# jing2li/MGPreconditionedGCR

Hardware: AMD Instinct MI355X
Metric: gcr_iterations_per_sec (higher is better)
Workload: dtype f64; 1 GPU; 3D 7-point Poisson 128^3 per GPU, unpreconditioned GCR restart 5, complex fp64, x0=0, RHS splitmix64 seed 0; rows=2097152, nnz=14581760, complex=True, stored_matrix_bytes=2097292, ell_width=7, tail_nnz=0, partition=1 GPU

## Files before the change

### mgpreconditionedgcr_amd/csrc/api.hip

```cpp
#include <algorithm>
#include <numeric>

#include <cstring>

#include "internal.h"

using namespace mgcr;

#define LOCK() std::lock_guard<std::recursive_mutex> lk__(ctx().mtx)

extern "C" {

int mgcr_csr_create(int64_t nrow, int64_t ncol, const int64_t *rowptr, const int64_t *col, const double *val_ri,
                    mgcr_op_t *out) {
    MGCR_TRY(require_ctx());
    MGCR_CHECK(out && rowptr && (col || rowptr[nrow] == 0) && (val_ri || rowptr[nrow] == 0), MGCR_ERR_INVALID,
               "mgcr_csr_create: null argument");
    LOCK();
    mgcr_op_s *op = new mgcr_op_s();
    op->kind = OP_CSR;
    op->dim = ncol;
    op->nrow = nrow;
    int rc = csr_build_device(nrow, ncol, rowptr, col, val_ri, &op->csr);
    if (rc != MGCR_OK) { delete op; return rc; }
// ... 168 lines not shown
    if (x_window) *x_window = o->csr.win_h;
    return MGCR_OK;
}

int mgcr_op_xr_fuse_kind(mgcr_op_t op, int32_t *kind) {
    MGCR_CHECK(op && kind, MGCR_ERR_INVALID, "mgcr_op_xr_fuse_kind: null argument");
    const Op *o = op_matrix(op);
    MGCR_CHECK(o->kind == OP_CSR, MGCR_ERR_UNSUPPORTED, "mgcr_op_xr_fuse_kind: not a Sparse");
    *kind = csr_fusable(o->csr, o->dist) ? csr_xr_fuse_kind(o->csr, o->dist) : 0;
    return MGCR_OK;
}

int mgcr_op_halo_kind(mgcr_op_t op, int32_t *kind) {
    MGCR_CHECK(op && kind, MGCR_ERR_INVALID, "mgcr_op_halo_kind: null argument");
    const Op *o = op_matrix(op);
    MGCR_CHECK(o->dist, MGCR_ERR_UNSUPPORTED, "mgcr_op_halo_kind: not a distributed Sparse");
    *kind = dist_halo_kind(o->dist);
    return MGCR_OK;
}

int mgcr_set_option(const char *name, int value, int *previous) {
    MGCR_CHECK(name, MGCR_ERR_INVALID, "null option name");
    if (!strcmp(name, "spmv_part")) {
        const int p = set_spmv_part(value);
        if (previous) *previous = p;
        return MGCR_OK;
    }
    bool prev;
    if (!strcmp(name, "pattern_storage")) prev = set_patterns_enabled(value != 0);
    else if (!strcmp(name, "stencil_storage")) prev = set_stencil_enabled(value != 0);
    else if (!strcmp(name, "lean_cycles")) prev = set_lean_enabled(value != 0);
    else if (!strcmp(name, "fused_apply")) prev = set_fuse_enabled(value != 0);
    else if (!strcmp(name, "graph_replay")) prev = set_graph_enabled(value != 0);
    else if (!strcmp(name, "resident_solver")) prev = set_resident_enabled(value != 0);
    else if (!strcmp(name, "step_build")) prev = set_stepbuild_enabled(value != 0);
    else if (!strcmp(name, "start_build")) prev = set_start_build_enabled(value != 0);
    else if (!strcmp(name, "step_build_keep_r")) {
        static bool last = true;
        prev = last;
        last = value != 0;
    }
    else if (!strcmp(name, "step_build_keep_all")) prev = set_stepbuild_keep_all_enabled(value != 0);
    else if (!strcmp(name, "halo_split")) prev = set_halo_split(value != 0);
    else if (!strcmp(name, "pw_tail")) prev = set_pw_tail_enabled(value != 0);
    else { set_error("mgcr_set_option: unknown option '%s'", name); return MGCR_ERR_INVALID; }
    if (previous) *previous = prev ? 1 : 0;
    return MGCR_OK;
}

int mgcr_stat(const char *name, int64_t *value) {
    MGCR_CHECK(name && value, MGCR_ERR_INVALID, "mgcr_stat: null argument");
    if (!strcmp(name, "resident_solves")) *value = resident_solve_count();
    else if (!strcmp(name, "step_build_launches")) *value = stepbuild_launch_count();
    else if (!strcmp(name, "start_build_launches")) *value = start_build_launch_count();
    else if (!strcmp(name, "small_solves")) *value = gcr_small_solve_count();
    else if (!strcmp(name, "one_launch_fallbacks")) *value = gcr_fallback_count();
    else if (!strcmp(name, "halo_split_exchanges")) *value = dist_halo_split_count();
    else if (!strcmp(name, "pw_tail_folds")) *value = comm_pw_tail_count();
    else if (!strcmp(name, "multi_solves")) *value = gcr_multi_solve_count();
    else if (!strcmp(name, "queue_solves")) *value = gcr_queue_stat(0);
    else if (!strcmp(name, "queue_admissions")) *value = gcr_queue_stat(1);
    else if (!strcmp(name, "queue_steps")) *value = gcr_queue_stat(2);
    else { set_error("mgcr_stat: unknown counter '%s'", name); return MGCR_ERR_INVALID; }
    return MGCR_OK;
}

int mgcr_selftest_coherence(int32_t steps, int32_t coherent, int64_t *rows_wrong) {
    MGCR_TRY(require_ctx());
    LOCK();
    return coherence_selftest(steps, coherent, rows_wrong);
}

int mgcr_op_stored_bytes(mgcr_op_t op, int64_t *matrix_bytes, int32_t *ell_width, int64_t *tail_nnz) {
    MGCR_CHECK(op, MGCR_ERR_INVALID, "null operator");
    const Op *o = op_matrix(op);
    if (o->kind == OP_CSR) {
        const CsrDev &A = o->csr;
        int64_t slab = (int64_t)A.nchunk * A.npad * A.L;
        int64_t ell_bytes = slab * (A.ell_val_re ? 12 : 20);
        if (csr_stencil_active(A)) ell_bytes = (A.npad / 64) * A.sten_stride * 8 + A.sten_kernel_ns * 20;
        else if (A.pat_mode == 1) ell_bytes = A.npad * 2 + (int64_t)A.npat * A.W * (A.pat_real ? 12 : 20);
        else if (A.pat_mode == 2) ell_bytes = A.npad * 2 + (int64_t)A.npat * A.W * 4 + slab * (A.ell_val_re ? 8 : 16);
        if (matrix_bytes) *matrix_bytes = ell_bytes + A.tail_nnz * 20 + A.n_tail_rows * 8 + (A.n_tail_rows ? 4 : 0);
        if (ell_width) *ell_width = A.nchunk * A.L;
        if (tail_nnz) *tail_nnz = A.tail_nnz;
        return MGCR_OK;
    }
    if (o->kind == OP_BCSR) {
        const BcsrDev &B = o->bcsr;
        if (matrix_bytes) *matrix_bytes = (int64_t)B.nblocks * (16LL * B.bs * B.bs + 4) + ((int64_t)B.nbrow + 1) * 4;
        if (ell_width) *ell_width = 0;
        if (tail_nnz) *tail_nnz = 0;
        return MGCR_OK;
    }
    set_error("mgcr_op_stored_bytes: not a matrix operator");
    return MGCR_ERR_UNSUPPORTED;
}

int mgcr_op_apply(mgcr_op_t op, mgcr_vec_t x, mgcr_vec_t y) {
    MGCR_TRY(require_ctx());
    MGCR_CHECK(op && x && y, MGCR_ERR_INVALID, "mgcr_op_apply: null argument");
    MGCR_REFUSE_MULTI_DIRAC(op, "mgcr_op_apply");
    MGCR_CHECK(x->n == op->dim, MGCR_ERR_INVALID, "Sparse matrix dimension does not match Field dimension!");
    int64_t nrow = op->nrow ? op->nrow : op->dim;
    MGCR_CHECK(y->n == nrow, MGCR_ERR_INVALID, "output Field has %lld entries, operator has %lld rows", (long long)y->n, (long long)nrow);
    MGCR_CHECK(x->d != y->d, MGCR_ERR_INVALID, "mgcr_op_apply: input and output must be different Fields");
// ... 233 lines not shown
```

### mgpreconditionedgcr_amd/csrc/gcr_stepbuild.hip

```cpp
#include <climits>
#include <cstdlib>
#include <type_traits>

#include "internal.h"
#include "reduce.h"
#include "gcr_dev.h"
#include "spmv_dev.h"
#include "exchange_dev.h"

namespace mgcr {

constexpr int SB_MAX_TRIPS = 4;
constexpr int SB_MAX_ND = 5;
constexpr int SB_KEEP_TB = 2;
template <int NDT> constexpr int sb_keep_rows() { return NDT == 1 ? 3 : 2; }
template <int NDT, bool XR, bool CLOSE> constexpr bool sb_close_merged() { return CLOSE && (NDT == 4 || (NDT == 5 && XR)); }

struct StepBuildArgs {
    RowMat m;
    const cplx *x;
    const cplx *aps[SB_MAX_ND];
    int64_t n;
    int nlogical;
    RowMap rm;
    DevState *st;
    int it;
    const double *partsR;
    int nblkR, strideR;
    double *hist;
    int hist_cap;
    const cplx *den;
    cplx *ap_out;
    double *partsA;
    LeanCoef *lc;
    const cplx *ps[SB_MAX_ND];
    cplx *p_out;
    cplx *xvec;
    cplx *xr_out;
    cplx *xr_den_slot;
    int xr_slot;
    double *partsR_out;
    v4i *slots;
    unsigned gen0;
    unsigned *abort_dev;
    int *abort_host;
    int spin_limit;
    int test_stall;
};

__device__ __forceinline__ cplx sb_xr_alpha(const ResSync &sy, DevState *st, LeanCoef *lc, cplx *xr_den_slot, int xr_slot, int lb) {
    const cplx num = make_double2(res_total(sy, 0), res_total(sy, 1)), den = make_double2(res_total(sy, 2), res_total(sy, 3));
    const cplx alpha = to_sgpr(cdiv(num, den));
    if (lb == 0 && threadIdx.x == 0) {
        *xr_den_slot = den;
        st->npend = xr_slot + 1;
    }
    if (lb == 0 && (int)threadIdx.x < LND) lean_pending_update(lc, xr_slot, alpha, (int)threadIdx.x);
    return alpha;
}

template <int MODE, int WT, int NDT, bool XR, bool CLOSE, bool REALC = false>
__global__ void __launch_bounds__(RED_THREADS, 8) step_build_kernel(StepBuildArgs a) {
    __shared__ double lds[(2 * NDT > 4 ? 2 * NDT : 4) * 17];
    __shared__ double lds_pw[2 * SB_MAX_ND * 17], lds_ws[2 * SB_MAX_ND * RES_GRP];
    __shared__ int gave_up;
    __shared__ cplx sbeta[NDT], scp[NDT];
    extern __shared__ __attribute__((aligned(16))) unsigned char sb_smem[];
    if (a.st->stop_at < a.st->base + a.it) return;
// ... 153 lines not shown
        }
        __builtin_amdgcn_sched_barrier(0);
    };
    if constexpr (XR) {
        if ((int)threadIdx.x < 4) {
            const v4i w4 = {__double2loint(mine), __double2hiint(mine), (int)sy.gen, 0};
            __builtin_amdgcn_raw_buffer_store_b128(w4, sy.slots, ((2 * RES_NV + (int)threadIdx.x) * RES_BLK + lb) * 16, 0, RES_SC1);
        }
        if constexpr (MERGED) close_last();
        const cplx xr0 = i0 < end ? a.x[i0] : make_double2(0., 0.);
        if (!res_collect<4>(sy, 2)) {
            res_abort(a.abort_dev, a.abort_host);
            for (int64_t i = i0; i < end; i += stride) a.xr_out[i] = make_double2(__builtin_nan(""), __builtin_nan(""));
            if (threadIdx.x == 0) a.partsR_out[lb] = __builtin_nan("");
            return;
        }
        if (ends_here) return;
        const cplx alpha = sb_xr_alpha(sy, a.st, a.lc, a.xr_den_slot, a.xr_slot, lb);
        double vr[1] = {0.};
        trip = 0;
        for (int64_t i = i0; i < end; i += stride, trip++) {
            const cplx rn = csub(i == i0 ? xr0 : a.x[i], cmul(alpha, arL[trip * RED_THREADS + (int)threadIdx.x]));
            a.xr_out[i] = rn;
            vr[0] += rn.x * rn.x + rn.y * rn.y;
        }
        const double tot = block_sum_owner<1>(vr, lds);
        if (threadIdx.x == 0) a.partsR_out[lb] = tot;
    }
}

template <class T>
__device__ __forceinline__ T *sb_elem(T *p, uint32_t off) {
    using C = std::conditional_t<std::is_const_v<T>, const char, char>;
    return reinterpret_cast<T *>(reinterpret_cast<C *>(p) + off);
}

__device__ __forceinline__ void sb_wave_pair_to_lds(double (&v)[2], double *lds, int k0) {
    double s;
    const int k = wave_multi_sum<2>(v, s);
    if (((int)threadIdx.x & 31) == 0) lds[(k0 + k) * 17 + ((int)threadIdx.x >> 6)] = s;
}
template <int NV>
__device__ __forceinline__ double sb_block_owner_from_lds(double *lds) {
    const int nwave = (blockDim.x + 63) >> 6;
    __syncthreads();
    double t = 0.;
    if (threadIdx.x < NV)
        for (int w = 0; w < nwave; w++) t += lds[threadIdx.x * 17 + w];
    return t;
}

template <int NDT, bool XR, bool CLOSE, bool REALC>
__global__ void __launch_bounds__(RED_THREADS, 8) step_keep_kernel(StepBuildArgs a) {
    __shared__ double lds[(2 * NDT > 4 ? 2 * NDT : 4) * 17];
    __shared__ double lds_pw[2 * SB_MAX_ND * 17], lds_ws[2 * SB_MAX_ND * RES_GRP];
    __shared__ int gave_up;
    __shared__ cplx sbeta[NDT], scp[NDT], scx[NDT];
    extern __shared__ __attribute__((aligned(16))) unsigned char sb_smem[];
    if (a.st->stop_at < a.st->base + a.it) return;
    const int lb = logical_workgroup(a.rm, (int)blockIdx.x, (int)gridDim.x);
    if (lb >= a.nlogical) return;
    cplx *arL = reinterpret_cast<cplx *>(sb_smem);
    const int tid = (int)threadIdx.x;
    ResSync sy;
    res_sync_init(sy, a.slots, a.gen0, a.nlogical, lb, a.abort_dev, a.spin_limit, lds_pw, lds_ws, &gave_up);
    if (a.test_stall && lb == a.test_stall - 1) return;
    int64_t i0, end, stride;
    row_range(a.rm, lb, a.nlogical, a.n, &i0, &end, &stride);
    auto row = [&](int t) -> int64_t { return i0 + (int64_t)t * stride; };
    uint32_t off[SB_MAX_TRIPS];
#pragma unroll
    for (int t = 0; t < SB_MAX_TRIPS; t++) off[t] = (uint32_t)row(t) * (uint32_t)sizeof(cplx);
    auto at = [&](auto *p, int t) { return sb_elem(p, off[t]); };
    cplx rk[SB_MAX_TRIPS];
#pragma unroll
    for (int t = 0; t < SB_MAX_TRIPS; t++) {
        const int64_t i = row(t);
        rk[t] = make_double2(0., 0.);
        if (i < end) {
            const PatLds pl{nullptr, nullptr, nullptr};
            cplx sum;
            const auto xj = [&](int32_t j) -> cplx { return *sb_elem(a.x, (uint32_t)j * (uint32_t)sizeof(cplx)); };
            if constexpr (REALC) sum = sten_row_product_t<7, false, 1>(a.m, i, xj);
            else sum = fused_row_product<3, 7>(a.m, i, 0, pl, xj);
            rk[t] = *at(a.x, t);
            arL[t * RED_THREADS + tid] = a.m.shift ? csub(rk[t], cmul(a.m.k, sum)) : sum;
        }
        __builtin_amdgcn_sched_barrier(0);
    }
    constexpr int KT = sb_keep_rows<NDT>();
    cplx pre[KT];
    {
#pragma unroll
        for (int jj = 0; jj < NDT; jj++) {
            const int j = NDT - 1 - jj;
            cplx b[SB_MAX_TRIPS];
#pragma unroll
            for (int t = 0; t < SB_MAX_TRIPS; t++) b[t] = row(t) < end ? ld_stream<true>(at(a.aps[j], t)) : make_double2(0., 0.);
            double v[2] = {0., 0.};
#pragma unroll
            for (int t = 0; t < SB_MAX_TRIPS; t++) {
                if (row(t) < end) {
                    const cplx tt = cconj_mul(arL[t * RED_THREADS + tid], b[t]);
                    v[0] += tt.x;
                    v[1] += tt.y;
                }
            }
            if (j == 0) {
#pragma unroll
                for (int u = 0; u < KT; u++) pre[u] = b[u];
            }
            sb_wave_pair_to_lds(v, lds, 2 * j);
            __builtin_amdgcn_sched_barrier(0);
        }
        const double mine = sb_block_owner_from_lds<2 * NDT>(lds);
        if (tid < 2 * NDT) {
            const v4i w4 = {__double2loint(mine), __double2hiint(mine), (int)sy.gen, 0};
            __builtin_amdgcn_raw_buffer_store_b128(w4, sy.slots, ((1 * RES_NV + tid) * RES_BLK + lb) * 16, 0, RES_SC1);
        }
    }
    if (!res_collect<2 * NDT>(sy, 1)) {
        res_abort(a.abort_dev, a.abort_host);
        for (int64_t i = i0; i < end; i += stride) a.ap_out[i] = make_double2(__builtin_nan(""), __builtin_nan(""));
        if (tid < 4) a.partsA[tid * RED_MAX_BLOCKS + lb] = __builtin_nan("");
        return;
    }
    bool ends_here = false;
    if (XR || lb == 0) {
        double rr[1];
        fold_partials<1>(a.partsR, a.nblkR, a.strideR, rr, lds);
        if (lb == 0 && threadIdx.x == 0) {
            close_step(a.st, a.it, rr[0], a.hist, a.hist_cap, CLOSE);
            if (CLOSE) a.st->closed = 1;
        }
        ends_here = __builtin_amdgcn_readfirstlane(!((rr[0] / a.st->bnorm2) > a.st->tol2)) != 0;
    }
    if (tid < NDT) sbeta[tid] = cdiv(make_double2(res_total(sy, 2 * tid), res_total(sy, 2 * tid + 1)), a.den[tid]);
    __syncthreads();
    if constexpr (CLOSE) {
        if (tid < NDT) {
            scp[tid] = lean_close_coef(a.lc, sbeta, NDT, tid);
            scx[tid] = a.lc->cx[tid];
        }
        __syncthreads();
    }
    if (!CLOSE && lb == 0 && tid <= NDT) lean_table_row<NDT>(a.lc, sbeta, tid);
    {
        cplx beta[NDT];
#pragma unroll
        for (int j = 0; j < NDT; j++) beta[j] = to_sgpr(sbeta[j]);
        double v[4] = {0., 0., 0., 0.};
#pragma unroll
        for (int t0 = 0; t0 < SB_MAX_TRIPS; t0 += SB_KEEP_TB) {
            cplx ac[SB_KEEP_TB];
#pragma unroll
            for (int u = 0; u < SB_KEEP_TB; u++) ac[u] = make_double2(0., 0.);
#pragma unroll
            for (int j = 0; j < NDT; j++) {
                cplx aj[SB_KEEP_TB];
#pragma unroll
                for (int u = 0; u < SB_KEEP_TB; u++)
                    aj[u] = (j == 0 && t0 + u < KT) ? pre[t0 + u < KT ? t0 + u : 0]
                            : row(t0 + u) < end   ? ld_stream<NTS>(at(a.aps[j], t0 + u))
                                                  : make_double2(0., 0.);
#pragma unroll
                for (int u = 0; u < SB_KEEP_TB; u++) ac[u] = csub(ac[u], cmul(beta[j], aj[u]));
                __builtin_amdgcn_sched_barrier(0);
            }
#pragma unroll
            for (int u = 0; u < SB_KEEP_TB; u++) {
                const int t = t0 + u;
                const int64_t i = row(t);
                if (i < end) {
                    const cplx an = cadd(arL[t * RED_THREADS + tid], ac[u]);
                    *at(a.ap_out, t) = an;
                    if (XR) arL[t * RED_THREADS + tid] = an;
                    const cplx tt = cconj_mul(rk[t], an);
                    v[0] += tt.x; v[1] += tt.y;
                    const cplx w = cconj_mul(an, an);
                    v[2] += w.x; v[3] += w.y;
                }
            }
        }
        const double mine = block_sum_owner<4>(v, lds);
        if (tid < 4) a.partsA[tid * RED_MAX_BLOCKS + lb] = mine;
        if (XR && tid < 4) {
            const v4i w4 = {__double2loint(mine), __double2hiint(mine), (int)sy.gen, 0};
            __builtin_amdgcn_raw_buffer_store_b128(w4, sy.slots, ((2 * RES_NV + tid) * RES_BLK + lb) * 16, 0, RES_SC1);
        }
    }
    if constexpr (CLOSE) {
        cplx cx[NDT], cp[NDT];
#pragma unroll
        for (int j = 0; j < NDT; j++) {
            cx[j] = to_sgpr(scx[j]);
            cp[j] = to_sgpr(scp[j]);
        }
#pragma unroll
        for (int t0 = 0; t0 < SB_MAX_TRIPS; t0 += SB_KEEP_TB) {
            cplx xv[SB_KEEP_TB], pc[SB_KEEP_TB];
#pragma unroll
            for (int u = 0; u < SB_KEEP_TB; u++) {
                xv[u] = row(t0 + u) < end ? *at(a.xvec, t0 + u) : make_double2(0., 0.);
                pc[u] = make_double2(0., 0.);
            }
#pragma unroll
            for (int j = 0; j < NDT; j++) {
                cplx pj[SB_KEEP_TB];
#pragma unroll
                for (int u = 0; u < SB_KEEP_TB; u++) pj[u] = row(t0 + u) < end ? ld_stream<NTS>(at(a.ps[j], t0 + u)) : make_double2(0., 0.);
#pragma unroll
                for (int u = 0; u < SB_KEEP_TB; u++) {
                    xv[u] = cadd(xv[u], cmul(cx[j], pj[u]));
                    pc[u] = csub(pc[u], cmul(cp[j], pj[u]));
                }
            }
#pragma unroll
            for (int u = 0; u < SB_KEEP_TB; u++) {
                const int64_t i = row(t0 + u);
                if (i < end) {
                    *at(a.xvec, t0 + u) = xv[u];
                    st_stream<NTS>(at(a.p_out, t0 + u), cadd(rk[t0 + u], pc[u]));
                }
            }
            __builtin_amdgcn_sched_barrier(0);
        }
    }
    if constexpr (XR) {
        if (!res_collect<4>(sy, 2)) {
            res_abort(a.abort_dev, a.abort_host);
            for (int64_t i = i0; i < end; i += stride) a.xr_out[i] = make_double2(__builtin_nan(""), __builtin_nan(""));
            if (threadIdx.x == 0) a.partsR_out[lb] = __builtin_nan("");
            return;
        }
        if (ends_here) return;
        const cplx alpha = sb_xr_alpha(sy, a.st, a.lc, a.xr_den_slot, a.xr_slot, lb);
        double vr[1] = {0.};
#pragma unroll
        for (int t = 0; t < SB_MAX_TRIPS; t++) {
            const int64_t i = row(t);
            if (i < end) {
                const cplx rn = csub(rk[t], cmul(alpha, arL[t * RED_THREADS + tid]));
                *at(a.xr_out, t) = rn;
                vr[0] += rn.x * rn.x + rn.y * rn.y;
            }
        }
        const double tot = block_sum_owner<1>(vr, lds);
        if (threadIdx.x == 0) a.partsR_out[lb] = tot;
    }
}

struct StartArgs {
    RowMat m;
    const cplx *b;
    cplx *ap0;
    int64_t n;
    int nlogical;
    RowMap rm;
    DevState *st;
    double *hist;
    LeanCoef *lc;
    cplx *den0;
    cplx *r_out;
    double *partsR_out;
    v4i *slots;
    unsigned gen0;
    unsigned *abort_dev;
    int *abort_host;
    int spin_limit;
    int test_stall;
};

template <bool REALC>
__global__ void __launch_bounds__(RED_THREADS, 8) start_build_kernel(StartArgs a) {
    __shared__ double lds[6 * 17];
    __shared__ double lds_pw[2 * SB_MAX_ND * 17], lds_ws[2 * SB_MAX_ND * RES_GRP];
    __shared__ int gave_up;
    extern __shared__ __attribute__((aligned(16))) unsigned char sb_smem[];
    if (a.st->stop_at < 0) return;
    const int lb = logical_workgroup(a.rm, (int)blockIdx.x, (int)gridDim.x);
    if (lb >= a.nlogical) return;
    cplx *apL = reinterpret_cast<cplx *>(sb_smem);
    ResSync sy;
    res_sync_init(sy, a.slots, a.gen0, a.nlogical, lb, a.abort_dev, a.spin_limit, lds_pw, lds_ws, &gave_up);
    if (a.test_stall && lb == a.test_stall - 1) return;
    int64_t i0, end, stride;
    row_range(a.rm, lb, a.nlogical, a.n, &i0, &end, &stride);
    {
        double v[6] = {0., 0., 0., 0., 0., 0.};
#pragma unroll
        for (int t = 0; t < SB_MAX_TRIPS; t++) {
            const int64_t i = i0 + (int64_t)t * stride;
            if (i < end) {
                const PatLds pl{nullptr, nullptr, nullptr};
                cplx sum;
                if constexpr (REALC) sum = sten_row_product_t<7, false, 1>(a.m, i, [&](int32_t j) -> cplx { return a.b[j]; });
                else sum = fused_row_product<3, 7>(a.m, i, 0, pl, [&](int32_t j) -> cplx { return a.b[j]; });
                const cplx rv = a.b[i];
                const cplx yi = a.m.shift ? csub(rv, cmul(a.m.k, sum)) : sum;
                a.ap0[i] = yi;
                apL[t * RED_THREADS + (int)threadIdx.x] = yi;
                v[4] += rv.x * rv.x + rv.y * rv.y;
                const cplx tt = cconj_mul(rv, yi);
                v[0] += tt.x; v[1] += tt.y;
                const cplx u = cconj_mul(yi, yi);
                v[2] += u.x; v[3] += u.y;
            }
            __builtin_amdgcn_sched_barrier(0);
        }
        const double mine = block_sum_owner<6>(v, lds);
        if ((int)threadIdx.x < 5) {
            const v4i w4 = {__double2loint(mine), __double2hiint(mine), (int)sy.gen, 0};
            __builtin_amdgcn_raw_buffer_store_b128(w4, sy.slots, ((1 * RES_NV + (int)threadIdx.x) * RES_BLK + lb) * 16, 0, RES_SC1);
        }
    }
    const cplx b0 = i0 < end ? a.b[i0] : make_double2(0., 0.);
    if (!res_collect<5>(sy, 1)) {
        res_abort(a.abort_dev, a.abort_host);
        for (int64_t i = i0; i < end; i += stride) a.r_out[i] = make_double2(__builtin_nan(""), __builtin_nan(""));
        if (threadIdx.x == 0) a.partsR_out[lb] = __builtin_nan("");
        return;
    }
    if (lb == 0 && threadIdx.x == 0) {
        const double nb = res_total(sy, 4);
        a.st->bnorm2 = nb;
        a.st->rr = nb;
        a.hist[0] = sqrt(nb) / sqrt(nb);
    }
    const cplx alpha = sb_xr_alpha(sy, a.st, a.lc, a.den0, 0, lb);
    double vr[1] = {0.};
#pragma unroll
    for (int t = 0; t < SB_MAX_TRIPS; t++) {
        const int64_t i = i0 + (int64_t)t * stride;
        if (i < end) {
            const cplx rn = csub(t == 0 ? b0 : a.b[i], cmul(alpha, apL[t * RED_THREADS + (int)threadIdx.x]));
            a.r_out[i] = rn;
            vr[0] += rn.x * rn.x + rn.y * rn.y;
        }
    }
    const double tot = block_sum_owner<1>(vr, lds);
    if (threadIdx.x == 0) a.partsR_out[lb] = tot;
}

static EnvSwitch g_stepbuild{"MGCR_STEPBUILD"}, g_start_build{"MGCR_START_BUILD"};
static EnvSwitch g_sb_keep_all{"MGCR_SB_KEEP_ALL"};
static EnvSwitch g_sb_real{"MGCR_SB_REAL"};
bool stepbuild_is_enabled() { return g_stepbuild.on(); }
bool set_stepbuild_enabled(bool on) { return g_stepbuild.set(on); }
bool set_start_build_enabled(bool on) { return g_start_build.set(on); }
bool set_stepbuild_keep_all_enabled(bool on) { return g_sb_keep_all.set(on); }
static int64_t g_stepbuild_launches = 0;
int64_t stepbuild_launch_count() { return g_stepbuild_launches; }

template <int NDT, bool XR, bool CLOSE> constexpr bool sb_keep_fits() { return NDT <= 2 || (NDT == 3 && !(XR && CLOSE)); }
template <int NDT, bool XR, bool CLOSE, bool R> const void *sb_keep() {
    if constexpr (sb_keep_fits<NDT, XR, CLOSE>()) return (const void *)step_keep_kernel<NDT, XR, CLOSE, R>;
    else return nullptr;
}
static const void *sb_kernel(int nd, bool xr, bool close, bool realc) {
    if (g_sb_keep_all.on() && nd <= 3) {
#define SKR(NDT, R) (close ? (xr ? sb_keep<NDT, true, true, R>() : sb_keep<NDT, false, true, R>()) \
                           : (xr ? sb_keep<NDT, true, false, R>() : sb_keep<NDT, false, false, R>()))
#define SKK(NDT) (realc ? SKR(NDT, true) : SKR(NDT, false))
        const void *keep = nd == 1 ? SKK(1) : nd == 2 ? SKK(2) : SKK(3);
#undef SKK
#undef SKR
        if (keep) return keep;
    }
#define SBR(NDT, R) (close ? (xr ? (const void *)step_build_kernel<3, 7, NDT, true, true, R> : (const void *)step_build_kernel<3, 7, NDT, false, true, R>) \
                           : (xr ? (const void *)step_build_kernel<3, 7, NDT, true, false, R> : (const void *)step_build_kernel<3, 7, NDT, false, false, R>))
#define SBK(NDT) (realc ? SBR(NDT, true) : SBR(NDT, false))
    switch (nd) {
        case 1: return SBK(1);
        case 2: return SBK(2);
        case 3: return SBK(3);
        case 4: return SBK(4);
        default: return SBK(5);
    }
#undef SBK
#undef SBR
}
bool launch_is_coresident(const void *kernel, int threads, size_t dyn_lds, int grid) {
    struct Key { const void *k; size_t lds; int threads; int per_cu; };
    static std::vector<Key> seen;
    int per_cu = -1;
    for (const Key &e : seen)
        if (e.k == kernel && e.lds == dyn_lds && e.threads == threads) per_cu = e.per_cu;
    if (per_cu < 0) {
        if (dyn_lds > 0) (void)hipFuncSetAttribute(kernel, hipFuncAttributeMaxDynamicSharedMemorySize, (int)(dyn_lds > 64 * 1024 ? dyn_lds : 64 * 1024));
        int nb = 0;
        if (hipOccupancyMaxActiveBlocksPerMultiprocessor(&nb, kernel, threads, dyn_lds) != hipSuccess) { (void)hipGetLastError(); nb = 0; }
        per_cu = nb;
        seen.push_back(Key{kernel, dyn_lds, threads, per_cu});
    }
    static const int force = getenv("MGCR_TEST_OCCUPANCY") ? atoi(getenv("MGCR_TEST_OCCUPANCY")) : -1;
    if (force >= 0) per_cu = force;
    return exchange_shared_init() == MGCR_OK && (int64_t)per_cu * exchange_shared().cus >= grid;
}

static size_t sb_lds_bytes(const CsrDev &A, int g) {
    return sizeof(cplx) * RED_THREADS * (size_t)((A.nrow + (int64_t)g * RED_THREADS - 1) / ((int64_t)g * RED_THREADS));
}

bool csr_step_build_eligible(const CsrDev &A, const DistCsr *dist, int lim) {
    if (!g_stepbuild.on() || dist || comm_live_count() > 0 || lim < 1 || lim > SB_MAX_ND) return false;
    if (!csr_fusable(A, nullptr) || !csr_stencil_active(A) || A.sten_rare || sten_slots(A) != 7) return false;
    const int g = red_grid(A.nrow);
    if (g < 64 || g % 8 != 0) return false;
    if ((int64_t)g * RED_THREADS * SB_MAX_TRIPS < A.nrow) return false;
    if (A.reach >= FUSED_TILE_REACH_DEFAULT) return false;
    if (exchange_shared_init() != MGCR_OK) return false;
    if (g > RES_BLK) return false;
    const size_t lds = sb_lds_bytes(A, g);
    const bool realc = g_sb_real.on() && row_mat(A, false, cplx{0., 0.}).realv;
    for (int xr = 0; xr < 2; xr++)
        for (int cl = 0; cl < 2; cl++)
            if (!launch_is_coresident(sb_kernel(lim, xr != 0, cl != 0, realc), RED_THREADS, lds, g)) return false;
    return true;
}

template <class Args>
static int sb_fill_common(Args &a, const CsrDev &A, bool shift, cplx k, DevState *st, const RowMap &rm, unsigned ngen) {
    MGCR_TRY(exchange_shared_init());
    const ExchangeShared &sh = exchange_shared();
    a.m = row_mat(A, shift, k);
    a.n = A.nrow;
    a.nlogical = red_grid(A.nrow);
    a.rm = rm;
    a.st = st;
    a.slots = sh.slots; a.abort_dev = sh.abort_dev; a.abort_host = sh.abort_host;
    a.gen0 = exchange_take_generations(ngen);
    a.test_stall = getenv("MGCR_TEST_STEPBUILD_STALL") ? atoi(getenv("MGCR_TEST_STEPBUILD_STALL")) : 0;
    a.spin_limit = getenv("MGCR_TEST_RESIDENT_SPIN_LIMIT") ? atoi(getenv("MGCR_TEST_RESIDENT_SPIN_LIMIT")) : RES_SPIN_LIMIT;
    return MGCR_OK;
}
static int sb_launch(const void *kernel, void *args, int grid, size_t lds_bytes, const char *who) {
    MGCR_CHECK(launch_is_coresident(kernel, RED_THREADS, lds_bytes, grid), MGCR_ERR_INVALID, "%s: launch would not be co-resident", who);
    void *kargs[1] = {args};
    MGCR_HIP(hipLaunchKernel(kernel, dim3((unsigned)grid), dim3(RED_THREADS), kargs, lds_bytes, ctx().stream));
    MGCR_HIP(hipGetLastError());
    return MGCR_OK;
}

int csr_step_build(const CsrDev &A, const cplx *x, bool shift, cplx k, const cplx *const *aps, int nd, DevState *st, int it, const double *partsR,
                   int nblkR, int strideR, double *hist, int hist_cap, const cplx *den, cplx *ap_out, double *partsA, LeanCoef *lc,
                   const RowMap &rm, cplx *xr_out, cplx *xr_den_slot, int xr_slot, double *partsR_out, const cplx *const *close_ps, cplx *close_p_out,
                   cplx *close_x) {
    MGCR_CHECK(nd >= 1 && nd <= SB_MAX_ND, MGCR_ERR_INVALID, "csr_step_build: 1..5 directions");
    StepBuildArgs a;
    MGCR_TRY(sb_fill_common(a, A, shift, k, st, rm, 3));
    a.x = x;
    for (int j = 0; j < SB_MAX_ND; j++) a.aps[j] = aps[j < nd ? j : 0];
    a.it = it; a.partsR = partsR; a.nblkR = nblkR; a.strideR = strideR; a.hist = hist; a.hist_cap = hist_cap;
    a.den = den; a.ap_out = ap_out; a.partsA = partsA; a.lc = lc;
    for (int j = 0; j < SB_MAX_ND; j++) a.ps[j] = close_ps ? close_ps[j < nd ? j : 0] : nullptr;
    a.p_out = close_p_out; a.xvec = close_x;
    a.xr_out = xr_out; a.xr_den_slot = xr_den_slot; a.xr_slot = xr_slot; a.partsR_out = partsR_out;
    MGCR_TRY(sb_launch(sb_kernel(nd, xr_out != nullptr, close_ps != nullptr, g_sb_real.on() && a.m.realv), &a, a.nlogical, sb_lds_bytes(A, a.nlogical),
                       "csr_step_build"));
    g_stepbuild_launches++;
    return MGCR_OK;
}

static int64_t g_start_build_launches = 0;
int64_t start_build_launch_count() { return g_start_build_launches; }
static const void *start_kernel(bool realc) {
    return realc ? (const void *)start_build_kernel<true> : (const void *)start_build_kernel<false>;
}

bool csr_start_build_eligible(const CsrDev &A, const DistCsr *dist) {
    if (!g_start_build.on() || !csr_step_build_eligible(A, dist, 1)) return false;
    const bool realc = g_sb_real.on() && row_mat(A, false, cplx{0., 0.}).realv;
    return launch_is_coresident(start_kernel(realc), RED_THREADS, sb_lds_bytes(A, red_grid(A.nrow)), red_grid(A.nrow));
}

int csr_start_build(const CsrDev &A, const cplx *b, bool shift, cplx k, cplx *ap0, DevState *st, double *hist, LeanCoef *lc, cplx *den0,
                    cplx *r_out, double *partsR_out, const RowMap &rm) {
    StartArgs a;
    MGCR_TRY(sb_fill_common(a, A, shift, k, st, rm, 1));
    a.b = b;
    a.ap0 = ap0;
    a.hist = hist; a.lc = lc; a.den0 = den0; a.r_out = r_out; a.partsR_out = partsR_out;
    MGCR_TRY(sb_launch(start_kernel(g_sb_real.on() && a.m.realv), &a, a.nlogical, sb_lds_bytes(A, a.nlogical), "csr_start_build"));
    g_start_build_launches++;
    return MGCR_OK;
}

}
```

### mgpreconditionedgcr_amd/csrc/internal.h

```cpp
#pragma once
#include <hip/hip_runtime.h>
#include <climits>
#include <cstdint>
#include <cstdio>
#include <cstdlib>
#include <cstring>
#include <mutex>
#include <string>
#include <type_traits>
#include <utility>
#include <vector>

#include "../../include/mgcr.h"

namespace mgcr {

typedef double2 cplx;

void set_error(const char *fmt, ...);
int hip_fail(hipError_t e, const char *what, const char *file, int line);

#define MGCR_HIP(call)                                                     \
    do {                                                                   \
        hipError_t e__ = (call);                                           \
// ... 159 lines not shown
    DevBuf() = default;
    DevBuf(DevBuf &&o) noexcept : p(o.release()) {}
    DevBuf &operator=(DevBuf &&o) noexcept { std::swap(p, o.p); return *this; }
    ~DevBuf() { if (p) hipFree(p); }
    hipError_t malloc(size_t count) { return hipMalloc((void **)&p, sizeof(T) * count); }
    bool alloc(size_t count) { return malloc(count) == hipSuccess; }
    T *release() { T *q = p; p = nullptr; return q; }
};

template <int LO, int HI, typename F>
static int dispatch_nd(int nd, F &&f) {
    if constexpr (LO < HI) {
        if (nd == LO) return f(std::integral_constant<int, LO>{});
        return dispatch_nd<LO + 1, HI>(nd, f);
    } else {
        return f(std::integral_constant<int, HI>{});
    }
}
template <int V0, int... VS, typename F>
static int dispatch_value(int v, F &&f) {
    if constexpr (sizeof...(VS) > 0) {
        if (v != V0) return dispatch_value<VS...>(v, f);
    }
    return f(std::integral_constant<int, V0>{});
}
template <typename F>
static int dispatch_bool(bool b, F &&f) { return b ? f(std::true_type{}) : f(std::false_type{}); }
template <typename... KA, typename... AA>
static int launch(void (*kernel)(KA...), unsigned grid, int block, size_t lds, AA... args) {
    hipLaunchKernelGGL(kernel, dim3(grid), dim3(block), lds, ctx().stream, args...);
    MGCR_HIP(hipGetLastError());
    return MGCR_OK;
}

int csr_build_device(int64_t nrow, int64_t ncol, const int64_t *h_rowptr, const int64_t *h_col,
                     const double *h_val_ri, CsrDev *out);
void csr_free(CsrDev *c);
bool set_patterns_enabled(bool on);
bool set_stencil_enabled(bool on);
bool stencil_enabled();
int ell_band_count(const CsrDev &A, unsigned long long *d_cnt);
bool csr_stencil_active(const CsrDev &A);
int set_spmv_part(int part);
bool set_lean_enabled(bool on);
bool set_fuse_enabled(bool on);
bool set_graph_enabled(bool on);
bool set_resident_enabled(bool on);
constexpr int MGCR_INT_GAVE_UP = 1001;
int resident_check(bool internal = false);
void resident_shutdown();
int64_t resident_solve_count();
bool set_stepbuild_enabled(bool on);
int64_t stepbuild_launch_count();
bool set_start_build_enabled(bool on);
int64_t start_build_launch_count();
bool set_stepbuild_keep_all_enabled(bool on);
int coherence_selftest(int steps, int coherent, int64_t *rows_wrong);
bool stepbuild_is_enabled();
bool launch_is_coresident(const void *kernel, int threads, size_t dyn_lds, int grid);
bool one_launch_paths_enabled();
int csr_apply(const CsrDev &A, const cplx *x, cplx *y, bool shift, cplx k, DistCsr *dist = nullptr, const cplx *w = nullptr);
bool csr_fusable(const CsrDev &A, const DistCsr *dist);
struct RowMap;
struct PwTail;
bool csr_step_apply_has_pw_tail(const CsrDev &A, const DistCsr *dist);
int csr_step_apply(const CsrDev &A, const cplx *x, cplx *y, bool shift, cplx k, const cplx *const *vecs, int nd, double *parts,
                   DistCsr *dist, const RowMap &rm, const PwTail *pw = nullptr);
struct DevState;
struct LeanCoef;
bool csr_xr_fusable(const CsrDev &A, const DistCsr *dist);
bool csr_apply_carry(const CsrDev &A, const cplx *x, cplx *y, bool shift, cplx k, const cplx *w);
int csr_xr_fuse_kind(const CsrDev &A, const DistCsr *dist);
int csr_step_apply_xr(const CsrDev &A, const cplx *r_in, const cplx *ap, cplx *r_out, cplx *y, bool shift, cplx k, const cplx *const *vecs,
                      int nd, double *parts, double *partsR, DevState *st, int it, const double *partsA, int nblkA, int strideA,
                      cplx *den_slot, int slot, LeanCoef *lc, const RowMap &rm);
int csr_init_apply(const CsrDev &A, const cplx *r0, cplx *aps0, bool shift, cplx k, const cplx *b, double *partsA, double *partsR,
                   double *partsN, DistCsr *dist, const RowMap &rm);
int bcsr_build_device(int32_t nbrow, int32_t nbcol, int32_t bs, const int32_t *h_browptr, const int32_t *h_bcol,
                      const double *h_blocks, BcsrDev *out);
void bcsr_free(BcsrDev *b);
int bcsr_apply(const BcsrDev &A, const cplx *x, cplx *y, const cplx *xh = nullptr, int32_t nb_own = INT32_MAX);

struct SkipRef {
    const int *p = nullptr;
    int it = 0;
};
void set_apply_skip(SkipRef s);
SkipRef get_apply_skip();

int dist_halo_begin(DistCsr *d, const cplx *x, bool overlap_interior = false);
int64_t dist_halo_split_count();
bool set_halo_split(bool on);
bool set_pw_tail_enabled(bool on);
int64_t comm_pw_tail_count();
int dist_halo_end(DistCsr *d);
bool dist_halo_overlaps();
const cplx *dist_halo_ptr(DistCsr *d);
int dist_halo_kind(DistCsr *d);
void dist_info(DistCsr *d, const cplx **xh, int64_t *interior_begin, int64_t *interior_end);
void dist_free(DistCsr *d);
Comm *dist_comm(DistCsr *d);
void dist_sizes(DistCsr *d, int64_t *nloc, int64_t *nh, int64_t *row0, int64_t *n_global, int *rank, int *nranks);
int comm_allreduce_host(Comm *c, double *buf, int64_t count);
int dist_exchange_rows_host(DistCsr *d, const double *own, int w, double *halo);
int dist_csr_create(Comm *c, int64_t n_global, int64_t row0, int64_t nloc, const int64_t *rowptr, const int64_t *col,
                    const double *val_ri, Op *op);
// ... 65 lines not shown
```

Before: 14780 it/s.

## Extend keep-all step-build kernel to 4/5 direction cases with register-lean policy

Moves the keep-all step-build kernel body into a shared include parameterized by a policy (trip batch, prefetch keep count, on-the-fly offsets). It adds a wide variant for nd=4 with XR and nd=5 with CLOSE. That variant uses a batch of one, no prefetched rows, and, for nd=5 with XR, offsets computed on the fly so it fits register limits. Those later GCR steps, which previously fell back to another path, can now use the fused keep-all kernel and avoid re-reading data. The risk is register pressure or spills in the wide kernel, and whether keep_all is on by default.

```diff
diff --git a/mgpreconditionedgcr_amd/csrc/api.hip b/mgpreconditionedgcr_amd/csrc/api.hip
--- a/mgpreconditionedgcr_amd/csrc/api.hip
+++ b/mgpreconditionedgcr_amd/csrc/api.hip
@@ -244,6 +244,7 @@
     MGCR_CHECK(name && value, MGCR_ERR_INVALID, "mgcr_stat: null argument");
     if (!strcmp(name, "resident_solves")) *value = resident_solve_count();
     else if (!strcmp(name, "step_build_launches")) *value = stepbuild_launch_count();
+    else if (!strcmp(name, "step_keep_wide_launches")) *value = stepbuild_keep_wide_launch_count();
     else if (!strcmp(name, "start_build_launches")) *value = start_build_launch_count();
     else if (!strcmp(name, "small_solves")) *value = gcr_small_solve_count();
     else if (!strcmp(name, "one_launch_fallbacks")) *value = gcr_fallback_count();
diff --git a/mgpreconditionedgcr_amd/csrc/gcr_stepbuild.hip b/mgpreconditionedgcr_amd/csrc/gcr_stepbuild.hip
--- a/mgpreconditionedgcr_amd/csrc/gcr_stepbuild.hip
+++ b/mgpreconditionedgcr_amd/csrc/gcr_stepbuild.hip
@@ -14,6 +14,10 @@
 constexpr int SB_MAX_ND = 5;
 constexpr int SB_KEEP_TB = 2;
 template <int NDT> constexpr int sb_keep_rows() { return NDT == 1 ? 3 : 2; }
+template <int TB_, int KT_, bool OTF_> struct SbKeepPolicy {
+    static constexpr int TB = TB_, KT = KT_;
+    static constexpr bool OTF = OTF_;
+};
 template <int NDT, bool XR, bool CLOSE> constexpr bool sb_close_merged() { return CLOSE && (NDT == 4 || (NDT == 5 && XR)); }
 
 struct StepBuildArgs {
@@ -273,202 +277,13 @@
 
 template <int NDT, bool XR, bool CLOSE, bool REALC>
 __global__ void __launch_bounds__(RED_THREADS, 8) step_keep_kernel(StepBuildArgs a) {
-    __shared__ double lds[(2 * NDT > 4 ? 2 * NDT : 4) * 17];
-    __shared__ double lds_pw[2 * SB_MAX_ND * 17], lds_ws[2 * SB_MAX_ND * RES_GRP];
-    __shared__ int gave_up;
-    __shared__ cplx sbeta[NDT], scp[NDT], scx[NDT];
-    extern __shared__ __attribute__((aligned(16))) unsigned char sb_smem[];
-    if (a.st->stop_at < a.st->base + a.it) return;
-    const int lb = logical_workgroup(a.rm, (int)blockIdx.x, (int)gridDim.x);
-    if (lb >= a.nlogical) return;
-    cplx *arL = reinterpret_cast<cplx *>(sb_smem);
-    const int tid = (int)threadIdx.x;
-    ResSync sy;
-    res_sync_init(sy, a.slots, a.gen0, a.nlogical, lb, a.abort_dev, a.spin_limit, lds_pw, lds_ws, &gave_up);
-    if (a.test_stall && lb == a.test_stall - 1) return;
-    int64_t i0, end, stride;
-    row_range(a.rm, lb, a.nlogical, a.n, &i0, &end, &stride);
-    auto row = [&](int t) -> int64_t { return i0 + (int64_t)t * stride; };
-    uint32_t off[SB_MAX_TRIPS];
-#pragma unroll
-    for (int t = 0; t < SB_MAX_TRIPS; t++) off[t] = (uint32_t)row(t) * (uint32_t)sizeof(cplx);
-    auto at = [&](auto *p, int t) { return sb_elem(p, off[t]); };
-    cplx rk[SB_MAX_TRIPS];
-#pragma unroll
-    for (int t = 0; t < SB_MAX_TRIPS; t++) {
-        const int64_t i = row(t);
-        rk[t] = make_double2(0., 0.);
-        if (i < end) {
-            const PatLds pl{nullptr, nullptr, nullptr};
-            cplx sum;
-            const auto xj = [&](int32_t j) -> cplx { return *sb_elem(a.x, (uint32_t)j * (uint32_t)sizeof(cplx)); };
-            if constexpr (REALC) sum = sten_row_product_t<7, false, 1>(a.m, i, xj);
-            else sum = fused_row_product<3, 7>(a.m, i, 0, pl, xj);
-            rk[t] = *at(a.x, t);
-            arL[t * RED_THREADS + tid] = a.m.shift ? csub(rk[t], cmul(a.m.k, sum)) : sum;
-        }
-        __builtin_amdgcn_sched_barrier(0);
-    }
-    constexpr int KT = sb_keep_rows<NDT>();
-    cplx pre[KT];
-    {
-#pragma unroll
-        for (int jj = 0; jj < NDT; jj++) {
-            const int j = NDT - 1 - jj;
-            cplx b[SB_MAX_TRIPS];
-#pragma unroll
-            for (int t = 0; t < SB_MAX_TRIPS; t++) b[t] = row(t) < end ? ld_stream<true>(at(a.aps[j], t)) : make_double2(0., 0.);
-            double v[2] = {0., 0.};
-#pragma unroll
-            for (int t = 0; t < SB_MAX_TRIPS; t++) {
-                if (row(t) < end) {
-                    const cplx tt = cconj_mul(arL[t * RED_THREADS + tid], b[t]);
-                    v[0] += tt.x;
-                    v[1] += tt.y;
-                }
-            }
-            if (j == 0) {
-#pragma unroll
-                for (int u = 0; u < KT; u++) pre[u] = b[u];
-            }
-            sb_wave_pair_to_lds(v, lds, 2 * j);
-            __builtin_amdgcn_sched_barrier(0);
-        }
-        const double mine = sb_block_owner_from_lds<2 * NDT>(lds);
-        if (tid < 2 * NDT) {
-            const v4i w4 = {__double2loint(mine), __double2hiint(mine), (int)sy.gen, 0};
-            __builtin_amdgcn_raw_buffer_store_b128(w4, sy.slots, ((1 * RES_NV + tid) * RES_BLK + lb) * 16, 0, RES_SC1);
-        }
-    }
-    if (!res_collect<2 * NDT>(sy, 1)) {
-        res_abort(a.abort_dev, a.abort_host);
-        for (int64_t i = i0; i < end; i += stride) a.ap_out[i] = make_double2(__builtin_nan(""), __builtin_nan(""));
-        if (tid < 4) a.partsA[tid * RED_MAX_BLOCKS + lb] = __builtin_nan("");
-        return;
-    }
-    bool ends_here = false;
-    if (XR || lb == 0) {
-        double rr[1];
-        fold_partials<1>(a.partsR, a.nblkR, a.strideR, rr, lds);
-        if (lb == 0 && threadIdx.x == 0) {
-            close_step(a.st, a.it, rr[0], a.hist, a.hist_cap, CLOSE);
-            if (CLOSE) a.st->closed = 1;
-        }
-        ends_here = __builtin_amdgcn_readfirstlane(!((rr[0] / a.st->bnorm2) > a.st->tol2)) != 0;
-    }
-    if (tid < NDT) sbeta[tid] = cdiv(make_double2(res_total(sy, 2 * tid), res_total(sy, 2 * tid + 1)), a.den[tid]);
-    __syncthreads();
-    if constexpr (CLOSE) {
-        if (tid < NDT) {
-            scp[tid] = lean_close_coef(a.lc, sbeta, NDT, tid);
-            scx[tid] = a.lc->cx[tid];
-        }
-        __syncthreads();
-    }
-    if (!CLOSE && lb == 0 && tid <= NDT) lean_table_row<NDT>(a.lc, sbeta, tid);
-    {
-        cplx beta[NDT];
-#pragma unroll
-        for (int j = 0; j < NDT; j++) beta[j] = to_sgpr(sbeta[j]);
-        double v[4] = {0., 0., 0., 0.};
-#pragma unroll
-        for (int t0 = 0; t0 < SB_MAX_TRIPS; t0 += SB_KEEP_TB) {
-            cplx ac[SB_KEEP_TB];
-#pragma unroll
-            for (int u = 0; u < SB_KEEP_TB; u++) ac[u] = make_double2(0., 0.);
-#pragma unroll
-            for (int j = 0; j < NDT; j++) {
-                cplx aj[SB_KEEP_TB];
-#pragma unroll
-                for (int u = 0; u < SB_KEEP_TB; u++)
-                    aj[u] = (j == 0 && t0 + u < KT) ? pre[t0 + u < KT ? t0 + u : 0]
-                            : row(t0 + u) < end   ? ld_stream<NTS>(at(a.aps[j], t0 + u))
-                                                  : make_double2(0., 0.);
-#pragma unroll
-                for (int u = 0; u < SB_KEEP_TB; u++) ac[u] = csub(ac[u], cmul(beta[j], aj[u]));
-                __builtin_amdgcn_sched_barrier(0);
-            }
-#pragma unroll
-            for (int u = 0; u < SB_KEEP_TB; u++) {
-                const int t = t0 + u;
-                const int64_t i = row(t);
-                if (i < end) {
-                    const cplx an = cadd(arL[t * RED_THREADS + tid], ac[u]);
-                    *at(a.ap_out, t) = an;
-                    if (XR) arL[t * RED_THREADS + tid] = an;
-                    const cplx tt = cconj_mul(rk[t], an);
-                    v[0] += tt.x; v[1] += tt.y;
-                    const cplx w = cconj_mul(an, an);
-                    v[2] += w.x; v[3] += w.y;
-                }
-            }
-        }
-        const double mine = block_sum_owner<4>(v, lds);
-        if (tid < 4) a.partsA[tid * RED_MAX_BLOCKS + lb] = mine;
-        if (XR && tid < 4) {
-            const v4i w4 = {__double2loint(mine), __double2hiint(mine), (int)sy.gen, 0};
-            __builtin_amdgcn_raw_buffer_store_b128(w4, sy.slots, ((2 * RES_NV + tid) * RES_BLK + lb) * 16, 0, RES_SC1);
-        }
-    }
-    if constexpr (CLOSE) {
-        cplx cx[NDT], cp[NDT];
-#pragma unroll
-        for (int j = 0; j < NDT; j++) {
-            cx[j] = to_sgpr(scx[j]);
-            cp[j] = to_sgpr(scp[j]);
-        }
-#pragma unroll
-        for (int t0 = 0; t0 < SB_MAX_TRIPS; t0 += SB_KEEP_TB) {
-            cplx xv[SB_KEEP_TB], pc[SB_KEEP_TB];
-#pragma unroll
-            for (int u = 0; u < SB_KEEP_TB; u++) {
-                xv[u] = row(t0 + u) < end ? *at(a.xvec, t0 + u) : make_double2(0., 0.);
-                pc[u] = make_double2(0., 0.);
-            }
-#pragma unroll
-            for (int j = 0; j < NDT; j++) {
-                cplx pj[SB_KEEP_TB];
-#pragma unroll
-                for (int u = 0; u < SB_KEEP_TB; u++) pj[u] = row(t0 + u) < end ? ld_stream<NTS>(at(a.ps[j], t0 + u)) : make_double2(0., 0.);
-#pragma unroll
-                for (int u = 0; u < SB_KEEP_TB; u++) {
-                    xv[u] = cadd(xv[u], cmul(cx[j], pj[u]));
-                    pc[u] = csub(pc[u], cmul(cp[j], pj[u]));
-                }
-            }
-#pragma unroll
-            for (int u = 0; u < SB_KEEP_TB; u++) {
-                const int64_t i = row(t0 + u);
-                if (i < end) {
-                    *at(a.xvec, t0 + u) = xv[u];
-                    st_stream<NTS>(at(a.p_out, t0 + u), cadd(rk[t0 + u], pc[u]));
-                }
-            }
-            __builtin_amdgcn_sched_barrier(0);
-        }
-    }
-    if constexpr (XR) {
-        if (!res_collect<4>(sy, 2)) {
-            res_abort(a.abort_dev, a.abort_host);
-            for (int64_t i = i0; i < end; i += stride) a.xr_out[i] = make_double2(__builtin_nan(""), __builtin_nan(""));
-            if (threadIdx.x == 0) a.partsR_out[lb] = __builtin_nan("");
-            return;
-        }
-        if (ends_here) return;
-        const cplx alpha = sb_xr_alpha(sy, a.st, a.lc, a.xr_den_slot, a.xr_slot, lb);
-        double vr[1] = {0.};
-#pragma unroll
-        for (int t = 0; t < SB_MAX_TRIPS; t++) {
-            const int64_t i = row(t);
-            if (i < end) {
-                const cplx rn = csub(rk[t], cmul(alpha, arL[t * RED_THREADS + tid]));
-                *at(a.xr_out, t) = rn;
-                vr[0] += rn.x * rn.x + rn.y * rn.y;
-            }
-        }
-        const double tot = block_sum_owner<1>(vr, lds);
-        if (threadIdx.x == 0) a.partsR_out[lb] = tot;
-    }
+    using POL = SbKeepPolicy<SB_KEEP_TB, sb_keep_rows<NDT>(), false>;
+#include "gcr_stepbuild_keep_body.h"
+}
+template <int NDT, bool XR, bool CLOSE, bool REALC>
+__global__ void __launch_bounds__(RED_THREADS, 8) step_keep_wide_kernel(StepBuildArgs a) {
+    using POL = SbKeepPolicy<1, 0, NDT == 5 && XR>;
+#include "gcr_stepbuild_keep_body.h"
 }
 
 struct StartArgs {
@@ -572,13 +387,31 @@
 bool set_stepbuild_keep_all_enabled(bool on) { return g_sb_keep_all.set(on); }
 static int64_t g_stepbuild_launches = 0;
 int64_t stepbuild_launch_count() { return g_stepbuild_launches; }
+static int64_t g_keep_wide_launches = 0;
+int64_t stepbuild_keep_wide_launch_count() { return g_keep_wide_launches; }
 
 template <int NDT, bool XR, bool CLOSE> constexpr bool sb_keep_fits() { return NDT <= 2 || (NDT == 3 && !(XR && CLOSE)); }
 template <int NDT, bool XR, bool CLOSE, bool R> const void *sb_keep() {
     if constexpr (sb_keep_fits<NDT, XR, CLOSE>()) return (const void *)step_keep_kernel<NDT, XR, CLOSE, R>;
     else return nullptr;
 }
+template <int NDT, bool XR, bool CLOSE> constexpr bool sb_keep_wide_fits() { return (NDT == 4 && XR) || (NDT == 5 && CLOSE); }
+template <int NDT, bool XR, bool CLOSE, bool R> const void *sb_keep_wide_form() {
+    if constexpr (sb_keep_wide_fits<NDT, XR, CLOSE>()) return (const void *)step_keep_wide_kernel<NDT, XR, CLOSE, R>;
+    else return nullptr;
+}
+static const void *sb_keep_wide(int nd, bool xr, bool close, bool realc) {
+#define SKR(NDT, R) (close ? (xr ? sb_keep_wide_form<NDT, true, true, R>() : sb_keep_wide_form<NDT, false, true, R>()) \
+                           : (xr ? sb_keep_wide_form<NDT, true, false, R>() : sb_keep_wide_form<NDT, false, false, R>()))
+#define SKK(NDT) (realc ? SKR(NDT, true) : SKR(NDT, false))
+    return nd == 4 ? SKK(4) : nd == 5 ? SKK(5) : nullptr;
+#undef SKK
+#undef SKR
+}
 static const void *sb_kernel(int nd, bool xr, bool close, bool realc) {
+    if (g_sb_keep_all.on() && nd > 3) {
+        if (const void *wide = sb_keep_wide(nd, xr, close, realc)) return wide;
+    }
     if (g_sb_keep_all.on() && nd <= 3) {
 #define SKR(NDT, R) (close ? (xr ? sb_keep<NDT, true, true, R>() : sb_keep<NDT, false, true, R>()) \
                            : (xr ? sb_keep<NDT, true, false, R>() : sb_keep<NDT, false, false, R>()))
@@ -677,9 +510,11 @@
     for (int j = 0; j < SB_MAX_ND; j++) a.ps[j] = close_ps ? close_ps[j < nd ? j : 0] : nullptr;
     a.p_out = close_p_out; a.xvec = close_x;
     a.xr_out = xr_out; a.xr_den_slot = xr_den_slot; a.xr_slot = xr_slot; a.partsR_out = partsR_out;
-    MGCR_TRY(sb_launch(sb_kernel(nd, xr_out != nullptr, close_ps != nullptr, g_sb_real.on() && a.m.realv), &a, a.nlogical, sb_lds_bytes(A, a.nlogical),
-                       "csr_step_build"));
+    const bool xr = xr_out != nullptr, close = close_ps != nullptr, realc = g_sb_real.on() && a.m.realv;
+    const void *kernel = sb_kernel(nd, xr, close, realc);
+    MGCR_TRY(sb_launch(kernel, &a, a.nlogical, sb_lds_bytes(A, a.nlogical), "csr_step_build"));
     g_stepbuild_launches++;
+    if (nd > 3 && kernel == sb_keep_wide(nd, xr, close, realc)) g_keep_wide_launches++;
     return MGCR_OK;
 }
 
diff --git a/mgpreconditionedgcr_amd/csrc/gcr_stepbuild_keep_body.h b/mgpreconditionedgcr_amd/csrc/gcr_stepbuild_keep_body.h
--- /dev/null
+++ b/mgpreconditionedgcr_amd/csrc/gcr_stepbuild_keep_body.h
@@ -0,0 +1,203 @@
+    constexpr int TB = POL::TB, KT = POL::KT;
+    constexpr bool OTF = POL::OTF;
+    __shared__ double lds[(2 * NDT > 4 ? 2 * NDT : 4) * 17];
+    __shared__ double lds_pw[2 * SB_MAX_ND * 17], lds_ws[2 * SB_MAX_ND * RES_GRP];
+    __shared__ int gave_up;
+    __shared__ cplx sbeta[NDT], scp[NDT], scx[NDT];
+    extern __shared__ __attribute__((aligned(16))) unsigned char sb_smem[];
+    if (a.st->stop_at < a.st->base + a.it) return;
+    const int lb = logical_workgroup(a.rm, (int)blockIdx.x, (int)gridDim.x);
+    if (lb >= a.nlogical) return;
+    cplx *arL = reinterpret_cast<cplx *>(sb_smem);
+    const int tid = (int)threadIdx.x;
+    ResSync sy;
+    res_sync_init(sy, a.slots, a.gen0, a.nlogical, lb, a.abort_dev, a.spin_limit, lds_pw, lds_ws, &gave_up);
+    if (a.test_stall && lb == a.test_stall - 1) return;
+    int64_t i0, end, stride;
+    row_range(a.rm, lb, a.nlogical, a.n, &i0, &end, &stride);
+    auto row = [&](int t) -> int64_t { return i0 + (int64_t)t * stride; };
+    uint32_t off[OTF ? 1 : SB_MAX_TRIPS];
+#pragma unroll
+    for (int t = 0; t < (OTF ? 1 : SB_MAX_TRIPS); t++) off[t] = (uint32_t)row(t) * (uint32_t)sizeof(cplx);
+    const uint32_t soff = OTF ? (uint32_t)__builtin_amdgcn_readfirstlane((int)((uint32_t)stride * (uint32_t)sizeof(cplx))) : 0u;
+    auto at = [&](auto *p, int t) {
+        if constexpr (OTF) return sb_elem(p, off[0] + (uint32_t)t * soff);
+        else return sb_elem(p, off[t]);
+    };
+    cplx rk[SB_MAX_TRIPS];
+#pragma unroll
+    for (int t = 0; t < SB_MAX_TRIPS; t++) {
+        const int64_t i = row(t);
+        rk[t] = make_double2(0., 0.);
+        if (i < end) {
+            const PatLds pl{nullptr, nullptr, nullptr};
+            cplx sum;
+            const auto xj = [&](int32_t j) -> cplx { return *sb_elem(a.x, (uint32_t)j * (uint32_t)sizeof(cplx)); };
+            if constexpr (REALC) sum = sten_row_product_t<7, false, 1>(a.m, i, xj);
+            else sum = fused_row_product<3, 7>(a.m, i, 0, pl, xj);
+            rk[t] = *at(a.x, t);
+            arL[t * RED_THREADS + tid] = a.m.shift ? csub(rk[t], cmul(a.m.k, sum)) : sum;
+        }
+        __builtin_amdgcn_sched_barrier(0);
+    }
+    cplx pre[KT > 0 ? KT : 1];
+    {
+#pragma unroll
+        for (int jj = 0; jj < NDT; jj++) {
+            const int j = NDT - 1 - jj;
+            cplx b[SB_MAX_TRIPS];
+#pragma unroll
+            for (int t = 0; t < SB_MAX_TRIPS; t++) b[t] = row(t) < end ? ld_stream<true>(at(a.aps[j], t)) : make_double2(0., 0.);
+            double v[2] = {0., 0.};
+#pragma unroll
+            for (int t = 0; t < SB_MAX_TRIPS; t++) {
+                if (row(t) < end) {
+                    const cplx tt = cconj_mul(arL[t * RED_THREADS + tid], b[t]);
+                    v[0] += tt.x;
+                    v[1] += tt.y;
+                }
+            }
+            if constexpr (KT > 0) {
+                if (j == 0) {
+#pragma unroll
+                    for (int u = 0; u < KT; u++) pre[u] = b[u];
+                }
+            }
+            sb_wave_pair_to_lds(v, lds, 2 * j);
+            __builtin_amdgcn_sched_barrier(0);
+        }
+        const double mine = sb_block_owner_from_lds<2 * NDT>(lds);
+        if (tid < 2 * NDT) {
+            const v4i w4 = {__double2loint(mine), __double2hiint(mine), (int)sy.gen, 0};
+            __builtin_amdgcn_raw_buffer_store_b128(w4, sy.slots, ((1 * RES_NV + tid) * RES_BLK + lb) * 16, 0, RES_SC1);
+        }
+    }
+    if (!res_collect<2 * NDT>(sy, 1)) {
+        res_abort(a.abort_dev, a.abort_host);
+        for (int64_t i = i0; i < end; i += stride) a.ap_out[i] = make_double2(__builtin_nan(""), __builtin_nan(""));
+        if (tid < 4) a.partsA[tid * RED_MAX_BLOCKS + lb] = __builtin_nan("");
+        return;
+    }
+    bool ends_here = false;
+    if (XR || lb == 0) {
+        double rr[1];
+        fold_partials<1>(a.partsR, a.nblkR, a.strideR, rr, lds);
+        if (lb == 0 && threadIdx.x == 0) {
+            close_step(a.st, a.it, rr[0], a.hist, a.hist_cap, CLOSE);
+            if (CLOSE) a.st->closed = 1;
+        }
+        ends_here = __builtin_amdgcn_readfirstlane(!((rr[0] / a.st->bnorm2) > a.st->tol2)) != 0;
+    }
+    if (tid < NDT) sbeta[tid] = cdiv(make_double2(res_total(sy, 2 * tid), res_total(sy, 2 * tid + 1)), a.den[tid]);
+    __syncthreads();
+    if constexpr (CLOSE) {
+        if (tid < NDT) {
+            scp[tid] = lean_close_coef(a.lc, sbeta, NDT, tid);
+            scx[tid] = a.lc->cx[tid];
+        }
+        __syncthreads();
+    }
+    if (!CLOSE && lb == 0 && tid <= NDT) lean_table_row<NDT>(a.lc, sbeta, tid);
+    {
+        cplx beta[NDT];
+#pragma unroll
+        for (int j = 0; j < NDT; j++) beta[j] = to_sgpr(sbeta[j]);
+        double v[4] = {0., 0., 0., 0.};
+#pragma unroll
+        for (int t0 = 0; t0 < SB_MAX_TRIPS; t0 += TB) {
+            cplx ac[TB];
+#pragma unroll
+            for (int u = 0; u < TB; u++) ac[u] = make_double2(0., 0.);
+#pragma unroll
+            for (int j = 0; j < NDT; j++) {
+                cplx aj[TB];
+#pragma unroll
+                for (int u = 0; u < TB; u++)
+                    aj[u] = (j == 0 && t0 + u < KT) ? pre[t0 + u < KT ? t0 + u : 0]
+                            : row(t0 + u) < end   ? ld_stream<NTS>(at(a.aps[j], t0 + u))
+                                                  : make_double2(0., 0.);
+#pragma unroll
+                for (int u = 0; u < TB; u++) ac[u] = csub(ac[u], cmul(beta[j], aj[u]));
+                __builtin_amdgcn_sched_barrier(0);
+            }
+#pragma unroll
+            for (int u = 0; u < TB; u++) {
+                const int t = t0 + u;
+                const int64_t i = row(t);
+                if (i < end) {
+                    const cplx an = cadd(arL[t * RED_THREADS + tid], ac[u]);
+                    *at(a.ap_out, t) = an;
+                    if (XR) arL[t * RED_THREADS + tid] = an;
+                    const cplx tt = cconj_mul(rk[t], an);
+                    v[0] += tt.x; v[1] += tt.y;
+                    const cplx w = cconj_mul(an, an);
+                    v[2] += w.x; v[3] += w.y;
+                }
+            }
+        }
+        const double mine = block_sum_owner<4>(v, lds);
+        if (tid < 4) a.partsA[tid * RED_MAX_BLOCKS + lb] = mine;
+        if (XR && tid < 4) {
+            const v4i w4 = {__double2loint(mine), __double2hiint(mine), (int)sy.gen, 0};
+            __builtin_amdgcn_raw_buffer_store_b128(w4, sy.slots, ((2 * RES_NV + tid) * RES_BLK + lb) * 16, 0, RES_SC1);
+        }
+    }
+    if constexpr (CLOSE) {
+        cplx cx[NDT], cp[NDT];
+#pragma unroll
+        for (int j = 0; j < NDT; j++) {
+            cx[j] = to_sgpr(scx[j]);
+            cp[j] = to_sgpr(scp[j]);
+        }
+#pragma unroll
+        for (int t0 = 0; t0 < SB_MAX_TRIPS; t0 += TB) {
+            cplx xv[TB], pc[TB];
+#pragma unroll
+            for (int u = 0; u < TB; u++) {
+                xv[u] = row(t0 + u) < end ? *at(a.xvec, t0 + u) : make_double2(0., 0.);
+                pc[u] = make_double2(0., 0.);
+            }
+#pragma unroll
+            for (int j = 0; j < NDT; j++) {
+                cplx pj[TB];
+#pragma unroll
+                for (int u = 0; u < TB; u++) pj[u] = row(t0 + u) < end ? ld_stream<NTS>(at(a.ps[j], t0 + u)) : make_double2(0., 0.);
+#pragma unroll
+                for (int u = 0; u < TB; u++) {
+                    xv[u] = cadd(xv[u], cmul(cx[j], pj[u]));
+                    pc[u] = csub(pc[u], cmul(cp[j], pj[u]));
+                }
+            }
+#pragma unroll
+            for (int u = 0; u < TB; u++) {
+                const int64_t i = row(t0 + u);
+                if (i < end) {
+                    *at(a.xvec, t0 + u) = xv[u];
+                    st_stream<NTS>(at(a.p_out, t0 + u), cadd(rk[t0 + u], pc[u]));
+                }
+            }
+            __builtin_amdgcn_sched_barrier(0);
+        }
+    }
+    if constexpr (XR) {
+        if (!res_collect<4>(sy, 2)) {
+            res_abort(a.abort_dev, a.abort_host);
+            for (int64_t i = i0; i < end; i += stride) a.xr_out[i] = make_double2(__builtin_nan(""), __builtin_nan(""));
+            if (threadIdx.x == 0) a.partsR_out[lb] = __builtin_nan("");
+            return;
+        }
+        if (ends_here) return;
+        const cplx alpha = sb_xr_alpha(sy, a.st, a.lc, a.xr_den_slot, a.xr_slot, lb);
+        double vr[1] = {0.};
+#pragma unroll
+        for (int t = 0; t < SB_MAX_TRIPS; t++) {
+            const int64_t i = row(t);
+            if (i < end) {
+                const cplx rn = csub(rk[t], cmul(alpha, arL[t * RED_THREADS + tid]));
+                *at(a.xr_out, t) = rn;
+                vr[0] += rn.x * rn.x + rn.y * rn.y;
+            }
+        }
+        const double tot = block_sum_owner<1>(vr, lds);
+        if (threadIdx.x == 0) a.partsR_out[lb] = tot;
+    }
diff --git a/mgpreconditionedgcr_amd/csrc/internal.h b/mgpreconditionedgcr_amd/csrc/internal.h
--- a/mgpreconditionedgcr_amd/csrc/internal.h
+++ b/mgpreconditionedgcr_amd/csrc/internal.h
@@ -235,6 +235,7 @@
 int64_t resident_solve_count();
 bool set_stepbuild_enabled(bool on);
 int64_t stepbuild_launch_count();
+int64_t stepbuild_keep_wide_launch_count();
 bool set_start_build_enabled(bool on);
 int64_t start_build_launch_count();
 bool set_stepbuild_keep_all_enabled(bool on);
```

Result: faster. 15260 it/s (median of 6 runs) (+3.2%).
